# Visual-Behavior/aloception-oss

Hardware: AMD Instinct MI355X
Metric: frames/sec (whole node) DeformableDETR-R50 inference (higher is better)
Workload: dtype bf16; 1 GPU; DeformableDETR-R50 inference bf16, batch 8 synthetic 1333x800 frames per GPU, random-init weights; launch=hip-graph replay + eager inference(), per_gpu_batch=8, global_batch=8, parallelism=batch-sharded x1, no collective

## Files before the change

aloception-oss_amd/csrc/conv.hip:

```cpp
#include "common.hpp"

namespace alo {
namespace {

typedef __attribute__((ext_vector_type(8))) __bf16 bf16x8_t;
__device__ __forceinline__ bf16x8_t as_bf16x8(const u32x4& v) {
    union { u32x4 u; bf16x8_t b; } x;
    x.u = v;
    return x.b;
}

constexpr int kPix = 64;
constexpr int kThreads = 128;
constexpr int kOutStride = 64 * 2 + 16;
constexpr int kRedOffset = kPix * kOutStride;

template <int STRIDE>
struct Geo {
    static constexpr int kChunk = STRIDE == 1 ? 64 : 32;
    static constexpr int kBpt = kChunk / 32;
    static constexpr int kRun = STRIDE == 1 ? kPix + 2 : 2 * kPix + 1;
    static constexpr int kSlots = 3 * kRun;
    static constexpr int kPixStride = kChunk * 2 + 16;
    static constexpr int kPieces = kSlots * (kChunk / 8);
    static constexpr int kIters = (kPieces + kThreads - 1) / kThreads;
    static constexpr int kLds = kSlots * kPixStride;
    static_assert(kLds >= kRedOffset + 64 * 64 * 4, "the epilogue's staging aliases the halo");
};

struct ConvDims {
    int N, H, W, Ho, Wo, Cin, Cout;
    int tiles_per_image;
    int relu;
    int zsplit, cin_per_z;
};

struct WFrag { u32x4 v[2][2]; };

template <int STRIDE>
__device__ __forceinline__ int slot_pixel(int slot, int p0, const ConvDims& dm) {
    if (STRIDE == 1) {
        const int run = slot / Geo<1>::kRun, pix = slot - run * Geo<1>::kRun;
        const int q = p0 + (run - 1) * dm.W - 1 + pix;
        const int last = dm.H * dm.W - 1;
        return q < 0 ? 0 : (q > last ? last : q);
    }
    const int dy = slot / Geo<2>::kRun, r = slot - dy * Geo<2>::kRun;
    const int odd = r < kPix + 1 ? 1 : 0;
    int f = p0 + (odd ? r - 1 : r - (kPix + 1)) - (dy == 0 ? dm.Wo : 0);
    const int last = dm.Ho * dm.Wo - 1;
    f = f < 0 ? 0 : (f > last ? last : f);
    const int yp = f / dm.Wo, xp = f - yp * dm.Wo;
    int iy = 2 * yp + (dy == 1 ? 0 : 1), ix = 2 * xp + odd;
    iy = iy > dm.H - 1 ? dm.H - 1 : iy;
    ix = ix > dm.W - 1 ? dm.W - 1 : ix;
    return iy * dm.W + ix;
}

template <int STRIDE, bool KSPLIT>
__global__ void __launch_bounds__(kThreads, 2)
conv3x3_kernel(const bf16_t* __restrict__ X, const bf16_t* __restrict__ Wp, const bf16_t* __restrict__ bias,
               bf16_t* __restrict__ Y, float* __restrict__ partial, const ConvDims dm) {
    using G = Geo<STRIDE>;
    extern __shared__ __attribute__((aligned(16))) unsigned char smem[];
    unsigned char* const halo = smem;
    const int tid = threadIdx.x, wave = tid >> 6, lane = tid & 63;
    const int nl = lane & 31, kg = lane >> 5;
    const int HWo = dm.Ho * dm.Wo;
    const int col0 = KSPLIT ? blockIdx.y * 64 : blockIdx.y * 128 + wave * 64;
    const bool has_cols = col0 < dm.Cout;
    float* const bias_s = reinterpret_cast<float*>(smem + G::kLds);
    {
        const int c = (KSPLIT ? blockIdx.y * 64 : blockIdx.y * 128) + tid;
        bias_s[tid] = (bias != nullptr && c < dm.Cout && (!KSPLIT || tid < 64)) ? bf16_to_f32(bias[c].bits) : 0.f;
    }

    const int ntiles = dm.tiles_per_image * dm.N;
    const int per_xcd = (ntiles + 7) >> 3, xcd = blockIdx.x & 7, lanes_per_xcd = gridDim.x >> 3;
    const int tile_end = (xcd + 1) * per_xcd < ntiles ? (xcd + 1) * per_xcd : ntiles;
    int tile = xcd * per_xcd + (blockIdx.x >> 3);
    if (tile >= tile_end) return;

    const int ksteps_per_tap = dm.Cin / 16;
    const size_t ctile_stride = (size_t)9 * ksteps_per_tap * 512;
    const bf16_t* wfrag = Wp + (size_t)(col0 / 32) * ctile_stride + lane * 8;

    constexpr int kBatches = 9 * G::kBpt;
    const int my_batches = KSPLIT ? (kBatches - wave + 1) / 2 : kBatches;
    auto batch = [&](int i) { return KSPLIT ? wave + 2 * i : i; };

    u32x4 stage[G::kIters];
    auto load_halo = [&](int tl, int c0) {
        const int im = tl / dm.tiles_per_image, first = (tl - im * dm.tiles_per_image) * kPix;
        const bf16_t* ximg = X + (size_t)im * dm.H * dm.W * dm.Cin + c0;
#pragma unroll
        for (int it = 0; it < G::kIters; ++it) {
            const int i = tid + it * kThreads;
            const int piece = i % (G::kChunk / 8), slot = i / (G::kChunk / 8);
            if (i < G::kPieces)
                stage[it] = *reinterpret_cast<const u32x4*>(ximg + (size_t)slot_pixel<STRIDE>(slot, first, dm) * dm.Cin + piece * 8);
        }
    };
    const int cbeg = blockIdx.z * dm.cin_per_z, cend = cbeg + dm.cin_per_z;
    load_halo(tile, cbeg);

    for (; tile < tile_end; tile += lanes_per_xcd) {
        const int img = tile / dm.tiles_per_image;
        const int p0 = (tile - img * dm.tiles_per_image) * kPix;

        unsigned tapmask[2];
#pragma unroll
        for (int a = 0; a < 2; ++a) {
            const int q = p0 + 32 * a + nl;
            const int y = q / dm.Wo, x = q - y * dm.Wo;
            unsigned m = 0;
#pragma unroll
            for (int t = 0; t < 9; ++t) {
                const int yy = y * STRIDE + t / 3 - 1, xx = x * STRIDE + t % 3 - 1;
                if (q < HWo && yy >= 0 && yy < dm.H && xx >= 0 && xx < dm.W) m |= 1u << t;
            }
            tapmask[a] = m;
        }

        f32x16 acc[2][2];
#pragma unroll
        for (int a = 0; a < 2; ++a)
#pragma unroll
            for (int b = 0; b < 2; ++b)
#pragma unroll
                for (int i = 0; i < 16; ++i) acc[a][b][i] = 0.f;

        for (int c0 = cbeg; c0 < cend; c0 += G::kChunk) {
            auto load_w = [&](WFrag& f, int kb) {
                const bf16_t* p = wfrag + (size_t)((kb / G::kBpt) * ksteps_per_tap + c0 / 16 + 2 * (kb % G::kBpt)) * 512;
#pragma unroll
                for (int j = 0; j < 2; ++j)
#pragma unroll
                    for (int b = 0; b < 2; ++b)
                        f.v[j][b] = *reinterpret_cast<const u32x4*>(p + (size_t)j * 512 + b * ctile_stride);
            };
            auto compute = [&](const WFrag& f, int kb) {
                const int t = kb / G::kBpt, dy = t / 3, dx = t - 3 * dy;
                const int slot = STRIDE == 1 ? dy * G::kRun + dx : dy * G::kRun + (dx == 0 ? 0 : (dx == 1 ? kPix + 1 : 1));
                const bool ok0 = (tapmask[0] >> t) & 1u, ok1 = (tapmask[1] >> t) & 1u;
                const unsigned char* a_base = halo + (slot + nl) * G::kPixStride + kg * 16 + (kb % G::kBpt) * 64;
#pragma unroll
                for (int j = 0; j < 2; ++j) {
                    u32x4 a0 = *reinterpret_cast<const u32x4*>(a_base + j * 32);
                    u32x4 a1 = *reinterpret_cast<const u32x4*>(a_base + 32 * G::kPixStride + j * 32);
                    if (!ok0) a0 = u32x4{0u, 0u, 0u, 0u};
                    if (!ok1) a1 = u32x4{0u, 0u, 0u, 0u};
#pragma unroll
                    for (int b = 0; b < 2; ++b) {
                        acc[0][b] = __builtin_amdgcn_mfma_f32_32x32x16_bf16(as_bf16x8(f.v[j][b]), as_bf16x8(a0), acc[0][b], 0, 0, 0);
                        acc[1][b] = __builtin_amdgcn_mfma_f32_32x32x16_bf16(as_bf16x8(f.v[j][b]), as_bf16x8(a1), acc[1][b], 0, 0, 0);
                    }
                }
            };
            WFrag w0, w1;
            if (has_cols) load_w(w0, batch(0));

#pragma unroll
            for (int it = 0; it < G::kIters; ++it) {
                const int i = tid + it * kThreads;
                const int piece = i % (G::kChunk / 8), slot = i / (G::kChunk / 8);
                if (i < G::kPieces) *reinterpret_cast<u32x4*>(halo + slot * G::kPixStride + piece * 16) = stage[it];
            }
            __syncthreads();
            if (c0 + G::kChunk < cend) load_halo(tile, c0 + G::kChunk);
            else if (tile + lanes_per_xcd < tile_end) load_halo(tile + lanes_per_xcd, cbeg);

            if (has_cols) {
#pragma unroll 1
                for (int i = 0; i < my_batches; i += 2) {
                    if (i + 1 < my_batches) load_w(w1, batch(i + 1));
                    compute(w0, batch(i));
                    if (i + 2 < my_batches) load_w(w0, batch(i + 2));
                    if (i + 1 < my_batches) compute(w1, batch(i + 1));
                }
            }
            __syncthreads();
        }

        if (KSPLIT) {
            float* red = reinterpret_cast<float*>(smem + kRedOffset);
            if (wave == 1) {
#pragma unroll
                for (int a = 0; a < 2; ++a)
#pragma unroll
                    for (int b = 0; b < 2; ++b)
#pragma unroll
                        for (int r = 0; r < 16; ++r) red[((a * 2 + b) * 16 + r) * 64 + lane] = acc[a][b][r];
            }
            __syncthreads();
            if (wave == 0) {
#pragma unroll
                for (int a = 0; a < 2; ++a)
#pragma unroll
                    for (int b = 0; b < 2; ++b)
#pragma unroll
                        for (int r = 0; r < 16; ++r) acc[a][b][r] += red[((a * 2 + b) * 16 + r) * 64 + lane];
            }
        }

        if (!KSPLIT && dm.zsplit > 1) {
            if (has_cols) {
                float* pz = partial + ((size_t)blockIdx.z * dm.N + img) * HWo * dm.Cout + col0;
#pragma unroll
                for (int a = 0; a < 2; ++a) {
                    const int q = p0 + 32 * a + nl;
                    if (q < HWo) {
#pragma unroll
                        for (int b = 0; b < 2; ++b)
#pragma unroll
                            for (int qd = 0; qd < 4; ++qd)
                                *reinterpret_cast<f32x4*>(pz + (size_t)q * dm.Cout + 32 * b + 8 * qd + 4 * kg) =
                                    f32x4{acc[a][b][4 * qd], acc[a][b][4 * qd + 1], acc[a][b][4 * qd + 2], acc[a][b][4 * qd + 3]};
                    }
                }
            }
        } else if (has_cols && !(KSPLIT && wave == 1)) {
            unsigned char* const obuf = smem + (KSPLIT ? 0 : wave) * (kPix * kOutStride);
#pragma unroll
            for (int b = 0; b < 2; ++b)
#pragma unroll
                for (int q = 0; q < 4; ++q) {
                    const int c = 32 * b + 8 * q + 4 * kg;
                    const f32x4 bb = *reinterpret_cast<const f32x4*>(bias_s + (KSPLIT ? 0 : wave) * 64 + c);
#pragma unroll
                    for (int a = 0; a < 2; ++a) {
                        float v0 = acc[a][b][4 * q] + bb[0], v1 = acc[a][b][4 * q + 1] + bb[1];
                        float v2 = acc[a][b][4 * q + 2] + bb[2], v3 = acc[a][b][4 * q + 3] + bb[3];
                        if (dm.relu) { v0 = fmaxf(v0, 0.f); v1 = fmaxf(v1, 0.f); v2 = fmaxf(v2, 0.f); v3 = fmaxf(v3, 0.f); }
                        *reinterpret_cast<u32x2*>(obuf + (32 * a + nl) * kOutStride + c * 2) = u32x2{pack_bf16x2(v0, v1), pack_bf16x2(v2, v3)};
                    }
                }
            __builtin_amdgcn_fence(__ATOMIC_RELEASE, "wavefront");
            __builtin_amdgcn_wave_barrier();
            __builtin_amdgcn_fence(__ATOMIC_ACQUIRE, "wavefront");
#pragma unroll
            for (int pass = 0; pass < 8; ++pass) {
                const int row = pass * 8 + (lane >> 3);
                const int q = p0 + row;
                if (q < HWo)
                    *reinterpret_cast<u32x4*>(Y + ((size_t)img * HWo + q) * dm.Cout + col0 + (lane & 7) * 8) =
                        *reinterpret_cast<const u32x4*>(obuf + row * kOutStride + (lane & 7) * 16);
            }
        }
        __syncthreads();
    }
}

__global__ void __launch_bounds__(256)
conv_splitk_finalize_kernel(const float* __restrict__ partial, const bf16_t* __restrict__ bias, bf16_t* __restrict__ Y, long rows,
                            int Cout, int Z, int relu) {
    const long n8 = rows * (Cout / 8);
    for (long i = (long)blockIdx.x * 256 + threadIdx.x; i < n8; i += (long)gridDim.x * 256) {
        const long e = i * 8;
        const int c = (int)(e % Cout);
        float v[8];
#pragma unroll
        for (int j = 0; j < 8; ++j) v[j] = bias ? bf16_to_f32(bias[c + j].bits) : 0.f;
        for (int z = 0; z < Z; ++z) {
            const float* p = partial + (size_t)z * rows * Cout + e;
            const f32x4 a = *reinterpret_cast<const f32x4*>(p), b = *reinterpret_cast<const f32x4*>(p + 4);
#pragma unroll
            for (int j = 0; j < 4; ++j) { v[j] += a[j]; v[4 + j] += b[j]; }
        }
        if (relu)
#pragma unroll
            for (int j = 0; j < 8; ++j) v[j] = fmaxf(v[j], 0.f);
        *reinterpret_cast<u32x4*>(Y + e) = u32x4{pack_bf16x2(v[0], v[1]), pack_bf16x2(v[2], v[3]), pack_bf16x2(v[4], v[5]), pack_bf16x2(v[6], v[7])};
    }
}

int conv_zsplit(int ntiles, int Cin, int Cout) {
    if (Cout == 64) return 1;
    const int base = ntiles * ((Cout + 127) / 128);
    int z = 1;
    while (base * z * 2 <= 1024 && Cin % (z * 2 * 64) == 0 && Cin / (z * 2) >= 128) z *= 2;
    return z;
}

template <int STRIDE, bool KSPLIT>
hipError_t launch_conv(const void* x, const void* w, const void* bias, void* y, void* partial, const ConvDims& dm, hipStream_t stream) {
    const void* kern = reinterpret_cast<const void*>(conv3x3_kernel<STRIDE, KSPLIT>);
    constexpr int lds = Geo<STRIDE>::kLds + kThreads * 4;
    void* args[] = {&x, &w, &bias, &y, &partial, const_cast<ConvDims*>(&dm)};
    const unsigned gy = KSPLIT ? dm.Cout / 64 : (dm.Cout + 127) / 128;
    const int ntiles = dm.tiles_per_image * dm.N;
    int per_xcd = (ntiles + 7) / 8;
    if (per_xcd > 128) per_xcd = 128;
    return hipLaunchKernel(kern, dim3((unsigned)(8 * per_xcd), gy, (unsigned)dm.zsplit), dim3(kThreads), args, lds, stream);
}

}
}

using namespace alo;

extern "C" size_t alo_conv3x3_workspace_bytes(int N, int H, int W, int Cin, int Cout, int stride) {
    if (N <= 0 || H <= 0 || W <= 0 || Cin <= 0 || Cout <= 0 || (stride != 1 && stride != 2)) return 0;
    const long hwo = (long)((H - 1) / stride + 1) * ((W - 1) / stride + 1);
    const int z = conv_zsplit((int)((hwo + kPix - 1) / kPix) * N, Cin, Cout);
    return z > 1 ? (size_t)z * N * hwo * Cout * sizeof(float) : 0;
}

extern "C" int alo_conv3x3_nhwc(const void* x, const void* w_packed, const void* bias, void* y, void* workspace, int N, int H,
                                int W, int Cin, int Cout, int stride, int relu, int dtype, void* stream) {
    ALO_REQUIRE(x && w_packed && y, ALO_ERR_INVALID_ARGUMENT, "alo_conv3x3_nhwc: null pointer argument");
    ALO_REQUIRE(N > 0 && H > 0 && W > 0, ALO_ERR_INVALID_ARGUMENT, "alo_conv3x3_nhwc: N, H, W must be positive");
    ALO_REQUIRE(stride == 1 || stride == 2, ALO_ERR_UNSUPPORTED, "alo_conv3x3_nhwc: stride must be 1 or 2 (got %d)", stride);
    ALO_REQUIRE(Cin >= 64 && Cin % 64 == 0 && Cout >= 64 && Cout % 64 == 0, ALO_ERR_UNSUPPORTED,
                "alo_conv3x3_nhwc: Cin and Cout must be multiples of 64 (Cin=%d Cout=%d)", Cin, Cout);
    ALO_REQUIRE(dtype == ALO_BF16, ALO_ERR_UNSUPPORTED, "alo_conv3x3_nhwc: bf16 only (dtype %d)", dtype);
    ALO_REQUIRE((((uintptr_t)x | (uintptr_t)w_packed | (uintptr_t)y | (uintptr_t)workspace) & 15) == 0, ALO_ERR_INVALID_ARGUMENT,
                "alo_conv3x3_nhwc: pointers must be 16-byte aligned");
    ALO_REQUIRE((long)H * W < (1L << 24) && (long)N * H * W * (long)(Cin > Cout ? Cin : Cout) < (1L << 40), ALO_ERR_UNSUPPORTED,
                "alo_conv3x3_nhwc: image too large");
    ConvDims dm;
    dm.N = N; dm.H = H; dm.W = W; dm.Cin = Cin; dm.Cout = Cout; dm.relu = relu;
    dm.Ho = (H - 1) / stride + 1;
    dm.Wo = (W - 1) / stride + 1;
    dm.tiles_per_image = (dm.Ho * dm.Wo + kPix - 1) / kPix;
    dm.zsplit = workspace ? conv_zsplit(dm.tiles_per_image * N, Cin, Cout) : 1;
    dm.cin_per_z = Cin / dm.zsplit;
    hipStream_t s = static_cast<hipStream_t>(stream);
    const bool ksplit = Cout == 64;
    hipError_t e = stride == 1 ? (ksplit ? launch_conv<1, true>(x, w_packed, bias, y, workspace, dm, s) : launch_conv<1, false>(x, w_packed, bias, y, workspace, dm, s))
                               : (ksplit ? launch_conv<2, true>(x, w_packed, bias, y, workspace, dm, s) : launch_conv<2, false>(x, w_packed, bias, y, workspace, dm, s));
    if (e != hipSuccess) return fail(ALO_ERR_LAUNCH, "alo_conv3x3_nhwc: %s", hipGetErrorString(e));
    if (dm.zsplit > 1) {
        const long rows = (long)N * dm.Ho * dm.Wo;
        const float* part = static_cast<const float*>(workspace);
        int z = dm.zsplit;
        long blocks = (rows * (Cout / 8) + 255) / 256;
        if (blocks > 4096) blocks = 4096;
        void* args[] = {&part, &bias, &y, const_cast<long*>(&rows), &Cout, &z, &relu};
        e = hipLaunchKernel(reinterpret_cast<const void*>(conv_splitk_finalize_kernel), dim3((unsigned)blocks), dim3(256), args, 0, s);
        if (e != hipSuccess) return fail(ALO_ERR_LAUNCH, "alo_conv3x3_nhwc (finalize): %s", hipGetErrorString(e));
    }
    return check_launch("alo_conv3x3_nhwc");
}
```

Baseline: 855.2 frames/s.

## Add LDS-staged double-buffered 3x3 conv kernel for large stride-2 convolutions

Adds a new 256-thread implicit-GEMM 3x3 conv kernel that stages input halos and weight fragments into LDS with direct global-to-LDS DMA loads, double-buffered across taps, using 128x128 tiles. A routing function sends stride-2 convolutions with Cout a multiple of 128, no split-K and enough blocks to this kernel; all other shapes keep the existing register-staged kernel. The aim is to overlap global loads with MFMA work and reuse weights across a larger pixel tile. In exchange it uses more LDS per block and applies only to a narrow set of shapes, mainly the stride-2 3x3 convs in the ResNet stages.

```diff
diff --git a/aloception-oss_amd/csrc/conv.hip b/aloception-oss_amd/csrc/conv.hip
--- a/aloception-oss_amd/csrc/conv.hip
+++ b/aloception-oss_amd/csrc/conv.hip
@@ -9,6 +9,250 @@
     x.u = v;
     return x.b;
 }
+
+constexpr int kThreads = 256;
+constexpr int kOutStride = 64 * 2 + 16;
+
+template <int STRIDE, int WM>
+struct Tile {
+    static constexpr int kWN = 4 / WM;
+    static constexpr int kTM = 64 * WM, kTN = 64 * kWN;
+    static constexpr int kCH = STRIDE == 1 ? 64 : 32;
+    static constexpr int kKS = kCH / 16;
+    static constexpr int kP = kCH / 8;
+    static constexpr int kHalo = STRIDE == 1 ? kTM + 2 : 2 * kTM + 1;
+    static constexpr int kNH = (kHalo * kP + 63) / 64;
+    static constexpr int kNW = kKS * (kTN / 32);
+    static constexpr int kHaloBytes = kHalo * kCH * 2;
+    static constexpr int kWBytes = kNW * 1024;
+    static constexpr int kLds = 2 * kHaloBytes + 2 * kWBytes;
+    static_assert(kLds >= 4 * 64 * kOutStride, "the epilogue's staging aliases the stage buffers");
+    static_assert(kHaloBytes % 16 == 0, "16-byte aligned buffers");
+};
+
+struct ConvDims {
+    int N, H, W, Ho, Wo, Cin, Cout;
+    int tiles_per_image;
+    int relu;
+    int zsplit, cin_per_z;
+};
+
+template <int STRIDE, int TM>
+__device__ __forceinline__ int slot_pixel(int slot, int dy, int p0, const ConvDims& dm) {
+    if (STRIDE == 1) {
+        const int q = p0 + (dy - 1) * dm.W - 1 + slot;
+        const int last = dm.H * dm.W - 1;
+        return q < 0 ? 0 : (q > last ? last : q);
+    }
+    const int odd = slot < TM + 1 ? 1 : 0;
+    int f = p0 + (odd ? slot - 1 : slot - (TM + 1)) - (dy == 0 ? dm.Wo : 0);
+    const int last = dm.Ho * dm.Wo - 1;
+    f = f < 0 ? 0 : (f > last ? last : f);
+    const int yp = f / dm.Wo, xp = f - yp * dm.Wo;
+    int iy = 2 * yp + (dy == 1 ? 0 : 1), ix = 2 * xp + odd;
+    iy = iy > dm.H - 1 ? dm.H - 1 : iy;
+    ix = ix > dm.W - 1 ? dm.W - 1 : ix;
+    return iy * dm.W + ix;
+}
+
+template <int P>
+__device__ __forceinline__ int piece_pos(int slot, int piece) { return piece ^ ((slot / (16 / P)) & (P - 1)); }
+
+__device__ __forceinline__ void dma16(const bf16_t* src, unsigned char* lds_dst) {
+#if defined(__HIP_DEVICE_COMPILE__)
+    __builtin_amdgcn_global_load_lds(src, reinterpret_cast<u32x4*>(lds_dst), 16, 0, 0);
+#endif
+}
+
+__device__ __forceinline__ void dma_wait_barrier(int n) {
+#define ALO_WAIT(N) asm volatile("s_waitcnt vmcnt(" #N ") lgkmcnt(0)\n\ts_barrier" ::: "memory")
+    switch (n) {
+        case 0: ALO_WAIT(0); break;
+        case 1: ALO_WAIT(1); break;
+        case 2: ALO_WAIT(2); break;
+        case 3: ALO_WAIT(3); break;
+        case 4: ALO_WAIT(4); break;
+        case 5: ALO_WAIT(5); break;
+        case 6: ALO_WAIT(6); break;
+        case 7: ALO_WAIT(7); break;
+        case 8: ALO_WAIT(8); break;
+        default: ALO_WAIT(9); break;
+    }
+#undef ALO_WAIT
+}
+
+template <int STRIDE, int WM, bool PAIR>
+__global__ void __launch_bounds__(kThreads, 2)
+conv3x3_lds_kernel(const bf16_t* __restrict__ X, const bf16_t* __restrict__ Wp, const bf16_t* __restrict__ bias,
+                   bf16_t* __restrict__ Y, float* __restrict__ partial, const ConvDims dm) {
+    using T = Tile<STRIDE, WM>;
+    static_assert(T::kNH <= 4 * 9, "dma_wait_barrier covers up to 9 halo instructions per wave");
+    extern __shared__ __attribute__((aligned(16))) unsigned char smem[];
+    unsigned char* const hbuf = smem;
+    unsigned char* const wbuf = smem + 2 * T::kHaloBytes;
+    const int tid = threadIdx.x, lane = tid & 63;
+    const int wave = __builtin_amdgcn_readfirstlane(tid >> 6);
+    const int nl = lane & 31, kg = lane >> 5;
+    const int wm = wave % WM, wn = wave / WM;
+    const int HWo = dm.Ho * dm.Wo;
+
+    const int ncol = dm.Cout / T::kTN;
+    const unsigned lb = xcd_contiguous_block(blockIdx.x, gridDim.x);
+    const int ctile = lb % ncol, tile = lb / ncol;
+    const int img = tile / dm.tiles_per_image;
+    const int p0 = (tile - img * dm.tiles_per_image) * T::kTM;
+    const int col0 = ctile * T::kTN + wn * 64;
+    const int ksteps_per_tap = dm.Cin / 16;
+    const int cbeg = blockIdx.y * dm.cin_per_z;
+    const int nrows = dm.cin_per_z / T::kCH * 3;
+    const int ntaps = nrows * 3;
+
+    const int my_h = (T::kNH - wave + 3) / 4;
+    const bf16_t* const ximg = X + (size_t)img * dm.H * dm.W * dm.Cin + cbeg;
+    const bf16_t* const wcol = Wp + (size_t)(ctile * T::kTN / 32) * 9 * ksteps_per_tap * 512 + lane * 8 + cbeg / 16 * 512;
+    auto issue_halo = [&](int u) {
+        const int c = (u / 3) * T::kCH, dy = u % 3;
+        unsigned char* const buf = hbuf + (u & 1) * T::kHaloBytes;
+#pragma unroll
+        for (int e = 0; e < (T::kNH + 3) / 4; ++e) {
+            const int j = wave + 4 * e;
+            const int g = j * 64 + lane, slot = g / T::kP, pos = g - slot * T::kP;
+            if (j < T::kNH && slot < T::kHalo)
+                dma16(ximg + (size_t)slot_pixel<STRIDE, T::kTM>(slot, dy, p0, dm) * dm.Cin + c + piece_pos<T::kP>(slot, pos) * 8,
+                      buf + j * 1024);
+        }
+    };
+    auto issue_w = [&](int t) {
+        const int c = (t / 9) * T::kCH, tap = t % 9;
+        unsigned char* const buf = wbuf + (t & 1) * T::kWBytes;
+#pragma unroll
+        for (int e = 0; e < (T::kNW + 3) / 4; ++e) {
+            const int j = wave + 4 * e;
+            if (j < T::kNW) {
+                const int ks = j / (T::kTN / 32), ct = j - ks * (T::kTN / 32);
+                dma16(wcol + ((size_t)ct * 9 * ksteps_per_tap + tap * ksteps_per_tap + c / 16 + ks) * 512, buf + j * 1024);
+            }
+        }
+    };
+
+    unsigned tapmask[2];
+#pragma unroll
+    for (int a = 0; a < 2; ++a) {
+        const int q = p0 + 64 * wm + 32 * a + nl;
+        const int y = q / dm.Wo, x = q - y * dm.Wo;
+        unsigned m = 0;
+#pragma unroll
+        for (int t = 0; t < 9; ++t) {
+            const int yy = y * STRIDE + t / 3 - 1, xx = x * STRIDE + t % 3 - 1;
+            if (q < HWo && yy >= 0 && yy < dm.H && xx >= 0 && xx < dm.W) m |= 1u << t;
+        }
+        tapmask[a] = m;
+    }
+
+    f32x16 acc[PAIR ? 2 : 1][2][2];
+#pragma unroll
+    for (int h = 0; h < (PAIR ? 2 : 1); ++h)
+#pragma unroll
+        for (int a = 0; a < 2; ++a)
+#pragma unroll
+            for (int b = 0; b < 2; ++b)
+#pragma unroll
+                for (int i = 0; i < 16; ++i) acc[h][a][b][i] = 0.f;
+
+    issue_w(0);
+    issue_halo(0);
+    for (int t = 0; t < ntaps; ++t) {
+        const int u = t / 3, dx = t % 3, tap = t % 9;
+        dma_wait_barrier(dx == 1 && u + 1 < nrows ? my_h : 0);
+        if (t + 1 < ntaps) issue_w(t + 1);
+        if (dx == 0 && u + 1 < nrows) issue_halo(u + 1);
+
+        const unsigned char* const hb = hbuf + (u & 1) * T::kHaloBytes;
+        const unsigned char* const wb = wbuf + (t & 1) * T::kWBytes;
+        const int sbase = 64 * wm + (STRIDE == 1 ? dx : (dx == 0 ? 0 : (dx == 1 ? T::kTM + 1 : 1)));
+        const int h_tap = PAIR && STRIDE == 2 ? (tap & 1) : 0;
+#pragma unroll
+        for (int ks = 0; ks < T::kKS; ++ks) {
+            u32x4 af[2], bfr[2];
+#pragma unroll
+            for (int a = 0; a < 2; ++a) {
+                const int slot = sbase + 32 * a + nl;
+                af[a] = *reinterpret_cast<const u32x4*>(hb + (slot * T::kP + piece_pos<T::kP>(slot, 2 * ks + kg)) * 16);
+                if (!((tapmask[a] >> tap) & 1u)) af[a] = u32x4{0u, 0u, 0u, 0u};
+            }
+#pragma unroll
+            for (int b = 0; b < 2; ++b)
+                bfr[b] = *reinterpret_cast<const u32x4*>(wb + (ks * (T::kTN / 32) + wn * 2 + b) * 1024 + lane * 16);
+            const int h = PAIR ? (STRIDE == 1 ? ks / 2 : h_tap) : 0;
+#pragma unroll
+            for (int b = 0; b < 2; ++b)
+#pragma unroll
+                for (int a = 0; a < 2; ++a) {
+                    if (!PAIR || h == 0)
+                        acc[0][a][b] = __builtin_amdgcn_mfma_f32_32x32x16_bf16(as_bf16x8(bfr[b]), as_bf16x8(af[a]), acc[0][a][b], 0, 0, 0);
+                    else
+                        acc[PAIR ? 1 : 0][a][b] = __builtin_amdgcn_mfma_f32_32x32x16_bf16(as_bf16x8(bfr[b]), as_bf16x8(af[a]),
+                                                                                           acc[PAIR ? 1 : 0][a][b], 0, 0, 0);
+                }
+        }
+    }
+    dma_wait_barrier(0);
+    if (PAIR)
+#pragma unroll
+        for (int a = 0; a < 2; ++a)
+#pragma unroll
+            for (int b = 0; b < 2; ++b)
+#pragma unroll
+                for (int i = 0; i < 16; ++i) acc[0][a][b][i] += acc[PAIR ? 1 : 0][a][b][i];
+
+    if (dm.zsplit > 1) {
+        float* pz = partial + ((size_t)blockIdx.y * dm.N + img) * HWo * dm.Cout + col0;
+#pragma unroll
+        for (int a = 0; a < 2; ++a) {
+            const int q = p0 + 64 * wm + 32 * a + nl;
+            if (q < HWo) {
+#pragma unroll
+                for (int b = 0; b < 2; ++b)
+#pragma unroll
+                    for (int qd = 0; qd < 4; ++qd)
+                        *reinterpret_cast<f32x4*>(pz + (size_t)q * dm.Cout + 32 * b + 8 * qd + 4 * kg) =
+                            f32x4{acc[0][a][b][4 * qd], acc[0][a][b][4 * qd + 1], acc[0][a][b][4 * qd + 2], acc[0][a][b][4 * qd + 3]};
+            }
+        }
+        return;
+    }
+    unsigned char* const obuf = smem + wave * (64 * kOutStride);
+#pragma unroll
+    for (int b = 0; b < 2; ++b)
+#pragma unroll
+        for (int q = 0; q < 4; ++q) {
+            const int c = 32 * b + 8 * q + 4 * kg;
+            float bb[4] = {0.f, 0.f, 0.f, 0.f};
+            if (bias != nullptr)
+#pragma unroll
+                for (int i = 0; i < 4; ++i) bb[i] = bf16_to_f32(bias[col0 + c + i].bits);
+#pragma unroll
+            for (int a = 0; a < 2; ++a) {
+                float v0 = acc[0][a][b][4 * q] + bb[0], v1 = acc[0][a][b][4 * q + 1] + bb[1];
+                float v2 = acc[0][a][b][4 * q + 2] + bb[2], v3 = acc[0][a][b][4 * q + 3] + bb[3];
+                if (dm.relu) { v0 = fmaxf(v0, 0.f); v1 = fmaxf(v1, 0.f); v2 = fmaxf(v2, 0.f); v3 = fmaxf(v3, 0.f); }
+                *reinterpret_cast<u32x2*>(obuf + (32 * a + nl) * kOutStride + c * 2) = u32x2{pack_bf16x2(v0, v1), pack_bf16x2(v2, v3)};
+            }
+        }
+    __builtin_amdgcn_fence(__ATOMIC_RELEASE, "wavefront");
+    __builtin_amdgcn_wave_barrier();
+    __builtin_amdgcn_fence(__ATOMIC_ACQUIRE, "wavefront");
+#pragma unroll
+    for (int pass = 0; pass < 8; ++pass) {
+        const int row = pass * 8 + (lane >> 3);
+        const int q = p0 + 64 * wm + row;
+        if (q < HWo)
+            *reinterpret_cast<u32x4*>(Y + ((size_t)img * HWo + q) * dm.Cout + col0 + (lane & 7) * 8) =
+                *reinterpret_cast<const u32x4*>(obuf + row * kOutStride + (lane & 7) * 16);
+    }
+}
+
+namespace regstage {
 
 constexpr int kPix = 64;
 constexpr int kThreads = 128;
@@ -26,13 +270,6 @@
     static constexpr int kIters = (kPieces + kThreads - 1) / kThreads;
     static constexpr int kLds = kSlots * kPixStride;
     static_assert(kLds >= kRedOffset + 64 * 64 * 4, "the epilogue's staging aliases the halo");
-};
-
-struct ConvDims {
-    int N, H, W, Ho, Wo, Cin, Cout;
-    int tiles_per_image;
-    int relu;
-    int zsplit, cin_per_z;
 };
 
 struct WFrag { u32x4 v[2][2]; };
@@ -251,37 +488,6 @@
     }
 }
 
-__global__ void __launch_bounds__(256)
-conv_splitk_finalize_kernel(const float* __restrict__ partial, const bf16_t* __restrict__ bias, bf16_t* __restrict__ Y, long rows,
-                            int Cout, int Z, int relu) {
-    const long n8 = rows * (Cout / 8);
-    for (long i = (long)blockIdx.x * 256 + threadIdx.x; i < n8; i += (long)gridDim.x * 256) {
-        const long e = i * 8;
-        const int c = (int)(e % Cout);
-        float v[8];
-#pragma unroll
-        for (int j = 0; j < 8; ++j) v[j] = bias ? bf16_to_f32(bias[c + j].bits) : 0.f;
-        for (int z = 0; z < Z; ++z) {
-            const float* p = partial + (size_t)z * rows * Cout + e;
-            const f32x4 a = *reinterpret_cast<const f32x4*>(p), b = *reinterpret_cast<const f32x4*>(p + 4);
-#pragma unroll
-            for (int j = 0; j < 4; ++j) { v[j] += a[j]; v[4 + j] += b[j]; }
-        }
-        if (relu)
-#pragma unroll
-            for (int j = 0; j < 8; ++j) v[j] = fmaxf(v[j], 0.f);
-        *reinterpret_cast<u32x4*>(Y + e) = u32x4{pack_bf16x2(v[0], v[1]), pack_bf16x2(v[2], v[3]), pack_bf16x2(v[4], v[5]), pack_bf16x2(v[6], v[7])};
-    }
-}
-
-int conv_zsplit(int ntiles, int Cin, int Cout) {
-    if (Cout == 64) return 1;
-    const int base = ntiles * ((Cout + 127) / 128);
-    int z = 1;
-    while (base * z * 2 <= 1024 && Cin % (z * 2 * 64) == 0 && Cin / (z * 2) >= 128) z *= 2;
-    return z;
-}
-
 template <int STRIDE, bool KSPLIT>
 hipError_t launch_conv(const void* x, const void* w, const void* bias, void* y, void* partial, const ConvDims& dm, hipStream_t stream) {
     const void* kern = reinterpret_cast<const void*>(conv3x3_kernel<STRIDE, KSPLIT>);
@@ -295,15 +501,70 @@
 }
 
 }
+
+__global__ void __launch_bounds__(256)
+conv_splitk_finalize_kernel(const float* __restrict__ partial, const bf16_t* __restrict__ bias, bf16_t* __restrict__ Y, long rows,
+                            int Cout, int Z, int relu) {
+    const long n8 = rows * (Cout / 8);
+    for (long i = (long)blockIdx.x * 256 + threadIdx.x; i < n8; i += (long)gridDim.x * 256) {
+        const long e = i * 8;
+        const int c = (int)(e % Cout);
+        float v[8];
+#pragma unroll
+        for (int j = 0; j < 8; ++j) v[j] = bias ? bf16_to_f32(bias[c + j].bits) : 0.f;
+        for (int z = 0; z < Z; ++z) {
+            const float* p = partial + (size_t)z * rows * Cout + e;
+            const f32x4 a = *reinterpret_cast<const f32x4*>(p), b = *reinterpret_cast<const f32x4*>(p + 4);
+#pragma unroll
+            for (int j = 0; j < 4; ++j) { v[j] += a[j]; v[4 + j] += b[j]; }
+        }
+        if (relu)
+#pragma unroll
+            for (int j = 0; j < 8; ++j) v[j] = fmaxf(v[j], 0.f);
+        *reinterpret_cast<u32x4*>(Y + e) = u32x4{pack_bf16x2(v[0], v[1]), pack_bf16x2(v[2], v[3]), pack_bf16x2(v[4], v[5]), pack_bf16x2(v[6], v[7])};
+    }
+}
+
+struct ConvRoute {
+    bool lds;
+    int tiles_per_image, zsplit;
+};
+
+ConvRoute conv_route(int N, int Ho, int Wo, int Cin, int Cout, int stride) {
+    ConvRoute r;
+    r.zsplit = 1;
+    if (Cout != 64) {
+        const long base = (long)((Ho * Wo + 63) / 64) * N * ((Cout + 127) / 128);
+        while (base * r.zsplit * 2 <= 1024 && Cin % (r.zsplit * 2 * 64) == 0 && Cin / (r.zsplit * 2) >= 128) r.zsplit *= 2;
+    }
+    const long lds_blocks = (long)((Ho * Wo + 127) / 128) * N * (Cout / 128);
+    r.lds = stride == 2 && Cout % 128 == 0 && r.zsplit == 1 && lds_blocks >= 512;
+    r.tiles_per_image = r.lds ? (Ho * Wo + 127) / 128 : (Ho * Wo + 63) / 64;
+    return r;
+}
+
+template <int STRIDE, int WM, bool PAIR>
+hipError_t launch_lds(const void* x, const void* w, const void* bias, void* y, void* partial, const ConvDims& dm, hipStream_t stream) {
+    using T = Tile<STRIDE, WM>;
+    const void* kern = reinterpret_cast<const void*>(conv3x3_lds_kernel<STRIDE, WM, PAIR>);
+    static unsigned long long lds_done = 0;
+    hipError_t e = ensure_dynamic_lds(kern, T::kLds, &lds_done);
+    if (e != hipSuccess) return e;
+    void* args[] = {&x, &w, &bias, &y, &partial, const_cast<ConvDims*>(&dm)};
+    const unsigned blocks = (unsigned)(dm.tiles_per_image * dm.N * (dm.Cout / T::kTN));
+    return hipLaunchKernel(kern, dim3(blocks, (unsigned)dm.zsplit), dim3(kThreads), args, T::kLds, stream);
+}
+
+}
 }
 
 using namespace alo;
 
 extern "C" size_t alo_conv3x3_workspace_bytes(int N, int H, int W, int Cin, int Cout, int stride) {
     if (N <= 0 || H <= 0 || W <= 0 || Cin <= 0 || Cout <= 0 || (stride != 1 && stride != 2)) return 0;
-    const long hwo = (long)((H - 1) / stride + 1) * ((W - 1) / stride + 1);
-    const int z = conv_zsplit((int)((hwo + kPix - 1) / kPix) * N, Cin, Cout);
-    return z > 1 ? (size_t)z * N * hwo * Cout * sizeof(float) : 0;
+    const int ho = (H - 1) / stride + 1, wo = (W - 1) / stride + 1;
+    const int z = conv_route(N, ho, wo, Cin, Cout, stride).zsplit;
+    return z > 1 ? (size_t)z * N * ho * wo * Cout * sizeof(float) : 0;
 }
 
 extern "C" int alo_conv3x3_nhwc(const void* x, const void* w_packed, const void* bias, void* y, void* workspace, int N, int H,
@@ -322,12 +583,15 @@
     dm.N = N; dm.H = H; dm.W = W; dm.Cin = Cin; dm.Cout = Cout; dm.relu = relu;
     dm.Ho = (H - 1) / stride + 1;
     dm.Wo = (W - 1) / stride + 1;
-    dm.tiles_per_image = (dm.Ho * dm.Wo + kPix - 1) / kPix;
-    dm.zsplit = workspace ? conv_zsplit(dm.tiles_per_image * N, Cin, Cout) : 1;
+    const ConvRoute rt = conv_route(N, dm.Ho, dm.Wo, Cin, Cout, stride);
+    dm.tiles_per_image = rt.tiles_per_image;
+    dm.zsplit = workspace ? rt.zsplit : 1;
     dm.cin_per_z = Cin / dm.zsplit;
     hipStream_t s = static_cast<hipStream_t>(stream);
     const bool ksplit = Cout == 64;
-    hipError_t e = stride == 1 ? (ksplit ? launch_conv<1, true>(x, w_packed, bias, y, workspace, dm, s) : launch_conv<1, false>(x, w_packed, bias, y, workspace, dm, s))
+    using regstage::launch_conv;
+    hipError_t e = rt.lds ? launch_lds<2, 2, false>(x, w_packed, bias, y, workspace, dm, s)
+                 : stride == 1 ? (ksplit ? launch_conv<1, true>(x, w_packed, bias, y, workspace, dm, s) : launch_conv<1, false>(x, w_packed, bias, y, workspace, dm, s))
                                : (ksplit ? launch_conv<2, true>(x, w_packed, bias, y, workspace, dm, s) : launch_conv<2, false>(x, w_packed, bias, y, workspace, dm, s));
     if (e != hipSuccess) return fail(ALO_ERR_LAUNCH, "alo_conv3x3_nhwc: %s", hipGetErrorString(e));
     if (dm.zsplit > 1) {
```

Result: no change. 859.2 frames/s (median of 6 runs) (+0.5%).

## Add four-wave 128-pixel conv3x3 kernel with weight register ring for Cout=64

Applied to the files above, without the earlier changes.

Adds a dedicated 3x3 convolution kernel for 64-output-channel layers. It uses 256-thread blocks and 128-pixel tiles, so each weight fragment feeds four MFMAs instead of two. Weight fragments are prefetched into a register ring eight k-steps ahead, and the next halo load is overlapped with compute. Two waves split the K reduction and combine partial sums through LDS. The old in-kernel KSPLIT path is removed, leaving the generic kernel for other channel counts. The gain is more reuse and better latency hiding, at the cost of higher register pressure and extra LDS traffic for the reduction.

```diff
diff --git a/aloception-oss_amd/csrc/conv.hip b/aloception-oss_amd/csrc/conv.hip
--- a/aloception-oss_amd/csrc/conv.hip
+++ b/aloception-oss_amd/csrc/conv.hip
@@ -13,7 +13,6 @@
 constexpr int kPix = 64;
 constexpr int kThreads = 128;
 constexpr int kOutStride = 64 * 2 + 16;
-constexpr int kRedOffset = kPix * kOutStride;
 
 template <int STRIDE>
 struct Geo {
@@ -25,7 +24,7 @@
     static constexpr int kPieces = kSlots * (kChunk / 8);
     static constexpr int kIters = (kPieces + kThreads - 1) / kThreads;
     static constexpr int kLds = kSlots * kPixStride;
-    static_assert(kLds >= kRedOffset + 64 * 64 * 4, "the epilogue's staging aliases the halo");
+    static_assert(kLds >= 2 * kPix * kOutStride, "the epilogue's staging aliases the halo");
 };
 
 struct ConvDims {
@@ -37,17 +36,18 @@
 
 struct WFrag { u32x4 v[2][2]; };
 
-template <int STRIDE>
+template <int STRIDE, int KPIX = kPix>
 __device__ __forceinline__ int slot_pixel(int slot, int p0, const ConvDims& dm) {
+    constexpr int kRun = STRIDE == 1 ? KPIX + 2 : 2 * KPIX + 1;
     if (STRIDE == 1) {
-        const int run = slot / Geo<1>::kRun, pix = slot - run * Geo<1>::kRun;
+        const int run = slot / kRun, pix = slot - run * kRun;
         const int q = p0 + (run - 1) * dm.W - 1 + pix;
         const int last = dm.H * dm.W - 1;
         return q < 0 ? 0 : (q > last ? last : q);
     }
-    const int dy = slot / Geo<2>::kRun, r = slot - dy * Geo<2>::kRun;
-    const int odd = r < kPix + 1 ? 1 : 0;
-    int f = p0 + (odd ? r - 1 : r - (kPix + 1)) - (dy == 0 ? dm.Wo : 0);
+    const int dy = slot / kRun, r = slot - dy * kRun;
+    const int odd = r < KPIX + 1 ? 1 : 0;
+    int f = p0 + (odd ? r - 1 : r - (KPIX + 1)) - (dy == 0 ? dm.Wo : 0);
     const int last = dm.Ho * dm.Wo - 1;
     f = f < 0 ? 0 : (f > last ? last : f);
     const int yp = f / dm.Wo, xp = f - yp * dm.Wo;
@@ -57,7 +57,7 @@
     return iy * dm.W + ix;
 }
 
-template <int STRIDE, bool KSPLIT>
+template <int STRIDE>
 __global__ void __launch_bounds__(kThreads, 2)
 conv3x3_kernel(const bf16_t* __restrict__ X, const bf16_t* __restrict__ Wp, const bf16_t* __restrict__ bias,
                bf16_t* __restrict__ Y, float* __restrict__ partial, const ConvDims dm) {
@@ -67,12 +67,12 @@
     const int tid = threadIdx.x, wave = tid >> 6, lane = tid & 63;
     const int nl = lane & 31, kg = lane >> 5;
     const int HWo = dm.Ho * dm.Wo;
-    const int col0 = KSPLIT ? blockIdx.y * 64 : blockIdx.y * 128 + wave * 64;
+    const int col0 = blockIdx.y * 128 + wave * 64;
     const bool has_cols = col0 < dm.Cout;
     float* const bias_s = reinterpret_cast<float*>(smem + G::kLds);
     {
-        const int c = (KSPLIT ? blockIdx.y * 64 : blockIdx.y * 128) + tid;
-        bias_s[tid] = (bias != nullptr && c < dm.Cout && (!KSPLIT || tid < 64)) ? bf16_to_f32(bias[c].bits) : 0.f;
+        const int c = blockIdx.y * 128 + tid;
+        bias_s[tid] = (bias != nullptr && c < dm.Cout) ? bf16_to_f32(bias[c].bits) : 0.f;
     }
 
     const int ntiles = dm.tiles_per_image * dm.N;
@@ -86,8 +86,6 @@
     const bf16_t* wfrag = Wp + (size_t)(col0 / 32) * ctile_stride + lane * 8;
 
     constexpr int kBatches = 9 * G::kBpt;
-    const int my_batches = KSPLIT ? (kBatches - wave + 1) / 2 : kBatches;
-    auto batch = [&](int i) { return KSPLIT ? wave + 2 * i : i; };
 
     u32x4 stage[G::kIters];
     auto load_halo = [&](int tl, int c0) {
@@ -158,7 +156,7 @@
                 }
             };
             WFrag w0, w1;
-            if (has_cols) load_w(w0, batch(0));
+            if (has_cols) load_w(w0, 0);
 
 #pragma unroll
             for (int it = 0; it < G::kIters; ++it) {
@@ -172,38 +170,17 @@
 
             if (has_cols) {
 #pragma unroll 1
-                for (int i = 0; i < my_batches; i += 2) {
-                    if (i + 1 < my_batches) load_w(w1, batch(i + 1));
-                    compute(w0, batch(i));
-                    if (i + 2 < my_batches) load_w(w0, batch(i + 2));
-                    if (i + 1 < my_batches) compute(w1, batch(i + 1));
+                for (int i = 0; i < kBatches; i += 2) {
+                    if (i + 1 < kBatches) load_w(w1, i + 1);
+                    compute(w0, i);
+                    if (i + 2 < kBatches) load_w(w0, i + 2);
+                    if (i + 1 < kBatches) compute(w1, i + 1);
                 }
             }
             __syncthreads();
         }
 
-        if (KSPLIT) {
-            float* red = reinterpret_cast<float*>(smem + kRedOffset);
-            if (wave == 1) {
-#pragma unroll
-                for (int a = 0; a < 2; ++a)
-#pragma unroll
-                    for (int b = 0; b < 2; ++b)
-#pragma unroll
-                        for (int r = 0; r < 16; ++r) red[((a * 2 + b) * 16 + r) * 64 + lane] = acc[a][b][r];
-            }
-            __syncthreads();
-            if (wave == 0) {
-#pragma unroll
-                for (int a = 0; a < 2; ++a)
-#pragma unroll
-                    for (int b = 0; b < 2; ++b)
-#pragma unroll
-                        for (int r = 0; r < 16; ++r) acc[a][b][r] += red[((a * 2 + b) * 16 + r) * 64 + lane];
-            }
-        }
-
-        if (!KSPLIT && dm.zsplit > 1) {
+        if (dm.zsplit > 1) {
             if (has_cols) {
                 float* pz = partial + ((size_t)blockIdx.z * dm.N + img) * HWo * dm.Cout + col0;
 #pragma unroll
@@ -219,14 +196,14 @@
                     }
                 }
             }
-        } else if (has_cols && !(KSPLIT && wave == 1)) {
-            unsigned char* const obuf = smem + (KSPLIT ? 0 : wave) * (kPix * kOutStride);
+        } else if (has_cols) {
+            unsigned char* const obuf = smem + wave * (kPix * kOutStride);
 #pragma unroll
             for (int b = 0; b < 2; ++b)
 #pragma unroll
                 for (int q = 0; q < 4; ++q) {
                     const int c = 32 * b + 8 * q + 4 * kg;
-                    const f32x4 bb = *reinterpret_cast<const f32x4*>(bias_s + (KSPLIT ? 0 : wave) * 64 + c);
+                    const f32x4 bb = *reinterpret_cast<const f32x4*>(bias_s + wave * 64 + c);
 #pragma unroll
                     for (int a = 0; a < 2; ++a) {
                         float v0 = acc[a][b][4 * q] + bb[0], v1 = acc[a][b][4 * q + 1] + bb[1];
@@ -251,6 +228,186 @@
     }
 }
 
+constexpr int kThreads4 = 256;
+constexpr int kPix4 = 128;
+constexpr int kDist = 8;
+
+template <int STRIDE, int NCOL>
+struct Geo4 {
+    static constexpr int kHalves = NCOL == 64 ? 2 : 1;
+    static constexpr int kChunk = STRIDE == 1 ? 64 : 32;
+    static constexpr int kSteps = kChunk / 16;
+    static constexpr int kKs = kHalves == 1 ? 9 * kSteps : (STRIDE == 1 ? 18 : 10);
+    static constexpr int kRing = kKs % 9 == 0 ? 9 : 10;
+    static constexpr int kRun = STRIDE == 1 ? kPix4 + 2 : 2 * kPix4 + 1;
+    static constexpr int kSlots = 3 * kRun;
+    static constexpr int kPixStride = kChunk * 2 + 16;
+    static constexpr int kPieces = kSlots * (kChunk / 8);
+    static constexpr int kIters = (kPieces + kThreads4 - 1) / kThreads4;
+    static constexpr int kLds = kSlots * kPixStride;
+    static constexpr int kOutStride = NCOL * 2 + 16;
+    static constexpr int kRedOffset = kPix4 * kOutStride;
+    static_assert(kLds >= kRedOffset + (kHalves == 2 ? 2 * 64 * 64 * 4 : 0), "the epilogue's staging aliases the halo");
+    static_assert(kIters <= 13, "register staging of the halo");
+    static_assert(kKs % kRing == 0 && kRing > kDist, "the weight ring");
+};
+
+template <int STRIDE, int NCOL>
+__global__ void __launch_bounds__(kThreads4, 2)
+conv3x3_kernel_w4(const bf16_t* __restrict__ X, const bf16_t* __restrict__ Wp, const bf16_t* __restrict__ bias,
+                  bf16_t* __restrict__ Y, const ConvDims dm) {
+    using G = Geo4<STRIDE, NCOL>;
+    extern __shared__ __attribute__((aligned(16))) unsigned char smem[];
+    unsigned char* const halo = smem;
+    const int tid = threadIdx.x, wave = tid >> 6, lane = tid & 63;
+    const int nl = lane & 31, kg = lane >> 5;
+    const int swave = __builtin_amdgcn_readfirstlane(wave);
+    const int wn = swave % (NCOL / 32), kh = swave / (NCOL / 32);
+    const int HWo = dm.Ho * dm.Wo;
+    const int col0 = blockIdx.y * NCOL + wn * 32;
+    float* const bias_s = reinterpret_cast<float*>(smem + G::kLds);
+    if (tid < NCOL) bias_s[tid] = bias != nullptr ? bf16_to_f32(bias[blockIdx.y * NCOL + tid].bits) : 0.f;
+
+    const int ntiles = dm.tiles_per_image * dm.N;
+    const int per_xcd = (ntiles + 7) >> 3, xcd = blockIdx.x & 7, lanes_per_xcd = gridDim.x >> 3;
+    const int tile_end = (xcd + 1) * per_xcd < ntiles ? (xcd + 1) * per_xcd : ntiles;
+    int tile = xcd * per_xcd + (blockIdx.x >> 3);
+    if (tile >= tile_end) return;
+
+    auto tap_of = [&](int j) {
+        return G::kHalves == 1 ? j / G::kSteps : (STRIDE == 1 ? j / 2 : 2 * (j / 2) + kh);
+    };
+    auto step_of = [&](int j) {
+        return G::kHalves == 1 ? j % G::kSteps : j % 2;
+    };
+    const int kh_step = G::kHalves == 2 && STRIDE == 1 ? 2 * kh : 0;
+    const int ksteps_per_tap = dm.Cin / 16;
+    const bf16_t* const wfrag = Wp + ((size_t)(col0 / 32) * 9 * ksteps_per_tap + kh_step) * 512 + lane * 8;
+    auto load_w = [&](int c0, int j) {
+        const int t = tap_of(j) < 9 ? tap_of(j) : 8;
+        return *reinterpret_cast<const u32x4*>(wfrag + (size_t)(t * ksteps_per_tap + c0 / 16 + step_of(j)) * 512);
+    };
+
+    u32x4 stage[G::kIters];
+    auto load_piece = [&](int it, int tl, int c0) {
+        const int i = tid + it * kThreads4;
+        const int piece = i % (G::kChunk / 8), slot = i / (G::kChunk / 8);
+        if (i < G::kPieces) {
+            const int im = tl / dm.tiles_per_image, first = (tl - im * dm.tiles_per_image) * kPix4;
+            const bf16_t* ximg = X + (size_t)im * dm.H * dm.W * dm.Cin + c0;
+            stage[it] = *reinterpret_cast<const u32x4*>(ximg + (size_t)slot_pixel<STRIDE, kPix4>(slot, first, dm) * dm.Cin + piece * 8);
+        }
+    };
+    const int cend = dm.Cin;
+#pragma unroll
+    for (int it = 0; it < G::kIters; ++it) load_piece(it, tile, 0);
+    u32x4 w[G::kRing];
+#pragma unroll
+    for (int j = 0; j < kDist; ++j) w[j] = load_w(0, j);
+
+    for (; tile < tile_end; tile += lanes_per_xcd) {
+        const int img = tile / dm.tiles_per_image;
+        const int p0 = (tile - img * dm.tiles_per_image) * kPix4;
+
+        unsigned tapmask[4];
+#pragma unroll
+        for (int a = 0; a < 4; ++a) {
+            const int q = p0 + 32 * a + nl;
+            const int y = q / dm.Wo, x = q - y * dm.Wo;
+            unsigned m = 0;
+#pragma unroll
+            for (int t = 0; t < 9; ++t) {
+                const int yy = y * STRIDE + t / 3 - 1, xx = x * STRIDE + t % 3 - 1;
+                if (q < HWo && yy >= 0 && yy < dm.H && xx >= 0 && xx < dm.W) m |= 1u << t;
+            }
+            tapmask[a] = m;
+        }
+
+        f32x16 acc[4];
+#pragma unroll
+        for (int a = 0; a < 4; ++a)
+#pragma unroll
+            for (int i = 0; i < 16; ++i) acc[a][i] = 0.f;
+
+        const unsigned char* const a_lane = halo + nl * G::kPixStride + kg * 16 + kh_step * 32;
+        for (int c0 = 0; c0 < cend; c0 += G::kChunk) {
+#pragma unroll
+            for (int it = 0; it < G::kIters; ++it) {
+                const int i = tid + it * kThreads4;
+                const int piece = i % (G::kChunk / 8), slot = i / (G::kChunk / 8);
+                if (i < G::kPieces) *reinterpret_cast<u32x4*>(halo + slot * G::kPixStride + piece * 16) = stage[it];
+            }
+            __syncthreads();
+
+            const bool last_chunk = c0 + G::kChunk >= cend;
+            const int c_next = last_chunk ? 0 : c0 + G::kChunk;
+            const int t_next = last_chunk ? tile + lanes_per_xcd : tile;
+            const bool halo_next = t_next < tile_end;
+#pragma unroll
+            for (int j = 0; j < G::kKs; ++j) {
+                w[(j + kDist) % G::kRing] = j + kDist < G::kKs ? load_w(c0, j + kDist) : load_w(c_next, j + kDist - G::kKs);
+                if (j == 0 && halo_next)
+#pragma unroll
+                    for (int it = 0; it < G::kIters; ++it) load_piece(it, t_next, c_next);
+
+                const int t = tap_of(j);
+                if (t < 9) {
+                    const int dy = t / 3, dx = t - 3 * dy;
+                    const int slot = STRIDE == 1 ? dy * G::kRun + dx : dy * G::kRun + (dx == 0 ? 0 : (dx == 1 ? kPix4 + 1 : 1));
+#pragma unroll
+                    for (int a = 0; a < 4; ++a) {
+                        u32x4 av = *reinterpret_cast<const u32x4*>(a_lane + (slot + 32 * a) * G::kPixStride + step_of(j) * 32);
+                        if (!((tapmask[a] >> t) & 1u)) av = u32x4{0u, 0u, 0u, 0u};
+                        acc[a] = __builtin_amdgcn_mfma_f32_32x32x16_bf16(as_bf16x8(w[j % G::kRing]), as_bf16x8(av), acc[a], 0, 0, 0);
+                    }
+                }
+            }
+            __syncthreads();
+        }
+
+        if (G::kHalves == 2) {
+            float* red = reinterpret_cast<float*>(smem + G::kRedOffset) + wn * 64 * 64;
+            if (kh == 1)
+#pragma unroll
+                for (int a = 0; a < 4; ++a)
+#pragma unroll
+                    for (int r = 0; r < 16; ++r) red[(a * 16 + r) * 64 + lane] = acc[a][r];
+            __syncthreads();
+            if (kh == 0)
+#pragma unroll
+                for (int a = 0; a < 4; ++a)
+#pragma unroll
+                    for (int r = 0; r < 16; ++r) acc[a][r] += red[(a * 16 + r) * 64 + lane];
+        }
+        if (kh == 0) {
+#pragma unroll
+            for (int q = 0; q < 4; ++q) {
+                const int c = wn * 32 + 8 * q + 4 * kg;
+                const f32x4 bb = *reinterpret_cast<const f32x4*>(bias_s + c);
+#pragma unroll
+                for (int a = 0; a < 4; ++a) {
+                    float v0 = acc[a][4 * q] + bb[0], v1 = acc[a][4 * q + 1] + bb[1];
+                    float v2 = acc[a][4 * q + 2] + bb[2], v3 = acc[a][4 * q + 3] + bb[3];
+                    if (dm.relu) { v0 = fmaxf(v0, 0.f); v1 = fmaxf(v1, 0.f); v2 = fmaxf(v2, 0.f); v3 = fmaxf(v3, 0.f); }
+                    *reinterpret_cast<u32x2*>(smem + (32 * a + nl) * G::kOutStride + c * 2) = u32x2{pack_bf16x2(v0, v1), pack_bf16x2(v2, v3)};
+                }
+            }
+        }
+        __syncthreads();
+        constexpr int kPerPix = NCOL / 8, kPass = kPix4 * kPerPix / kThreads4;
+#pragma unroll
+        for (int pass = 0; pass < kPass; ++pass) {
+            const int i = pass * kThreads4 + tid;
+            const int row = i / kPerPix, pc = i % kPerPix;
+            const int q = p0 + row;
+            if (q < HWo)
+                *reinterpret_cast<u32x4*>(Y + ((size_t)img * HWo + q) * dm.Cout + blockIdx.y * NCOL + pc * 8) =
+                    *reinterpret_cast<const u32x4*>(smem + row * G::kOutStride + pc * 16);
+        }
+        __syncthreads();
+    }
+}
+
 __global__ void __launch_bounds__(256)
 conv_splitk_finalize_kernel(const float* __restrict__ partial, const bf16_t* __restrict__ bias, bf16_t* __restrict__ Y, long rows,
                             int Cout, int Z, int relu) {
@@ -282,16 +439,27 @@
     return z;
 }
 
-template <int STRIDE, bool KSPLIT>
+template <int STRIDE>
 hipError_t launch_conv(const void* x, const void* w, const void* bias, void* y, void* partial, const ConvDims& dm, hipStream_t stream) {
-    const void* kern = reinterpret_cast<const void*>(conv3x3_kernel<STRIDE, KSPLIT>);
+    const void* kern = reinterpret_cast<const void*>(conv3x3_kernel<STRIDE>);
     constexpr int lds = Geo<STRIDE>::kLds + kThreads * 4;
     void* args[] = {&x, &w, &bias, &y, &partial, const_cast<ConvDims*>(&dm)};
-    const unsigned gy = KSPLIT ? dm.Cout / 64 : (dm.Cout + 127) / 128;
     const int ntiles = dm.tiles_per_image * dm.N;
     int per_xcd = (ntiles + 7) / 8;
     if (per_xcd > 128) per_xcd = 128;
-    return hipLaunchKernel(kern, dim3((unsigned)(8 * per_xcd), gy, (unsigned)dm.zsplit), dim3(kThreads), args, lds, stream);
+    return hipLaunchKernel(kern, dim3((unsigned)(8 * per_xcd), (unsigned)((dm.Cout + 127) / 128), (unsigned)dm.zsplit), dim3(kThreads),
+                           args, lds, stream);
+}
+
+template <int STRIDE, int NCOL>
+hipError_t launch_conv_w4(const void* x, const void* w, const void* bias, void* y, const ConvDims& dm, hipStream_t stream) {
+    const void* kern = reinterpret_cast<const void*>(conv3x3_kernel_w4<STRIDE, NCOL>);
+    constexpr int lds = Geo4<STRIDE, NCOL>::kLds + NCOL * 4;
+    void* args[] = {&x, &w, &bias, &y, const_cast<ConvDims*>(&dm)};
+    const int ntiles = dm.tiles_per_image * dm.N;
+    int per_xcd = (ntiles + 7) / 8;
+    if (per_xcd > 64) per_xcd = 64;
+    return hipLaunchKernel(kern, dim3((unsigned)(8 * per_xcd), (unsigned)(dm.Cout / NCOL)), dim3(kThreads4), args, lds, stream);
 }
 
 }
@@ -326,9 +494,13 @@
     dm.zsplit = workspace ? conv_zsplit(dm.tiles_per_image * N, Cin, Cout) : 1;
     dm.cin_per_z = Cin / dm.zsplit;
     hipStream_t s = static_cast<hipStream_t>(stream);
-    const bool ksplit = Cout == 64;
-    hipError_t e = stride == 1 ? (ksplit ? launch_conv<1, true>(x, w_packed, bias, y, workspace, dm, s) : launch_conv<1, false>(x, w_packed, bias, y, workspace, dm, s))
-                               : (ksplit ? launch_conv<2, true>(x, w_packed, bias, y, workspace, dm, s) : launch_conv<2, false>(x, w_packed, bias, y, workspace, dm, s));
+    hipError_t e;
+    if (Cout == 64) {
+        dm.tiles_per_image = (dm.Ho * dm.Wo + kPix4 - 1) / kPix4;
+        e = stride == 1 ? launch_conv_w4<1, 64>(x, w_packed, bias, y, dm, s) : launch_conv_w4<2, 64>(x, w_packed, bias, y, dm, s);
+    } else {
+        e = stride == 1 ? launch_conv<1>(x, w_packed, bias, y, workspace, dm, s) : launch_conv<2>(x, w_packed, bias, y, workspace, dm, s);
+    }
     if (e != hipSuccess) return fail(ALO_ERR_LAUNCH, "alo_conv3x3_nhwc: %s", hipGetErrorString(e));
     if (dm.zsplit > 1) {
         const long rows = (long)N * dm.Ho * dm.Wo;
```

After: 862.6 frames/s before, 869.7 frames/s after (median of 6 runs). Within noise of the previous version (+0.8%).
